# Ascend-Research/HeadPoseEstimation-WHENet

Hardware: NVIDIA H100
Metric: head-crops/sec @224x224 bf16 (higher is better)
Workload: dtype bf16

## Files before the change

### headposeestimation-whenet_b200/csrc/kernels_dwse.cuh

```cuda
#pragma once
#include <cuda.h>

#include "kernels_fused.cuh"

namespace whenet {
namespace fused {

struct alignas(64) DwSeParams {
    CUtensorMap tmE;
    CUtensorMap tmW;
    CUtensorMap tmX;
    CUtensorMap tmWx;
    const float* b_exp;
    const float* b_dw;
    int* tflag;
    void* out;
    float* partial;
    const float *w_se1t, *b_se1, *w_se2, *b_se2;
    float* gate;
    int Cse;
    float inv_hw;
    int se_tail;
    int scale_out;
    int C, pad;
    int n_chunks, chunks_per_cta;
    int N;
    int tiles_x, Ho_img;
};

template <int KS, int S, int HIN>
struct DwSeGeom {
    static constexpr int HO = (HIN + S - 1) / S;
    static constexpr int R = 7;
    static constexpr int SPR = HO / R;
    static constexpr int NSTRIPS = HO * SPR;
    static constexpr int PW = (HO - 1) * S + KS;
    static constexpr int NCOL = (R - 1) * S + KS;
};

template <int KS, int S, int HIN, int CC>
struct DwSeThreads { static constexpr int value = ((DwSeGeom<KS, S, HIN>::NSTRIPS * (CC / 4)) + 31) / 32 * 32; };

template <int KS, int S, int HIN, int CC>
constexpr size_t dwse_smem(int C, int Cse) {
    using G = DwSeGeom<KS, S, HIN>;
    return (size_t)2 * ((G::PW * G::PW * CC * 2 + 127) / 128 * 128)
           + (size_t)2 * ((CC * 4 + KS * KS * CC * 2 + 127) / 128 * 128)
           + (size_t)2 * G::NSTRIPS * CC * 4
           + (size_t)(C + Cse + 32) * 4 + 256;
}

template <typename T, int KS, int S, int HIN, int CC>
__device__ __forceinline__ void dw_strip(uint32_t erow, uint32_t cst, int cv, T* dst, int C, uint32_t red) {
    using G = DwSeGeom<KS, S, HIN>;
    constexpr int PITCH = CC * 2;
    const float4 bq = lds_f4(cst + (uint32_t)cv * 16);
    const uint32_t cst_h = cst + (uint32_t)(CC * 4 + cv * 8);
    __half2 hacc[G::R][2];
#pragma unroll
    for (int r = 0; r < G::R; ++r) { hacc[r][0] = __float2half2_rn(0.f); hacc[r][1] = __float2half2_rn(0.f); }
#pragma unroll
    for (int ky = 0; ky < KS; ++ky) {
        __half2 wr[KS][2];
#pragma unroll
        for (int kx = 0; kx < KS; ++kx) {
            uint32_t w0, w1;
            lds64(cst_h + (uint32_t)((ky * KS + kx) * CC) * 2, w0, w1);
            wr[kx][0] = *reinterpret_cast<__half2*>(&w0); wr[kx][1] = *reinterpret_cast<__half2*>(&w1);
        }
#pragma unroll
        for (int col = 0; col < G::NCOL; ++col) {
            uint32_t a, b;
            lds64(erow + (uint32_t)(col * PITCH), a, b);
            const __half2 x01 = *reinterpret_cast<__half2*>(&a), x23 = *reinterpret_cast<__half2*>(&b);
#pragma unroll
            for (int r = 0; r < G::R; ++r) {
                const int kx = col - r * S;
                if (kx >= 0 && kx < KS) {
                    hacc[r][0] = __hfma2(x01, wr[kx][0], hacc[r][0]);
                    hacc[r][1] = __hfma2(x23, wr[kx][1], hacc[r][1]);
                }
            }
        }
        erow += G::PW * PITCH;
    }
    const float2 sc = make_float2(kDwScale, kDwScale);
    float sum[4] = {0.f, 0.f, 0.f, 0.f};
#pragma unroll
    for (int r = 0; r < G::R; ++r) {
        float2 a0 = make_float2(bq.x, bq.y), a1 = make_float2(bq.z, bq.w);
        ffma2(a0, __half22float2(hacc[r][0]), sc);
        ffma2(a1, __half22float2(hacc[r][1]), sc);
        a0.x = swish_from_half(a0.x); a0.y = swish_from_half(a0.y);
        a1.x = swish_from_half(a1.x); a1.y = swish_from_half(a1.y);
        sum[0] += a0.x; sum[1] += a0.y; sum[2] += a1.x; sum[3] += a1.y;
        uint2 o;
        o.x = pack2<T>(a0.x, a0.y);
        o.y = pack2<T>(a1.x, a1.y);
        *reinterpret_cast<uint2*>(dst + (long long)r * C) = o;
    }
    asm volatile("st.shared.v4.f32 [%0], {%1,%2,%3,%4};" ::"r"(red), "f"(sum[0]), "f"(sum[1]), "f"(sum[2]), "f"(sum[3]) : "memory");
}

template <int NSTRIPS, int CC>
__device__ __forceinline__ void squeeze_sums(uint32_t red, float* dst, float* means, float inv_hw, int lane) {
    for (int cc = lane; cc < CC; cc += 32) {
        const uint32_t r0 = red + (uint32_t)(cc * 4);
        float s4[4] = {0.f, 0.f, 0.f, 0.f};
#pragma unroll
        for (int y = 0; y < NSTRIPS; ++y) {
            float t;
            asm volatile("ld.shared.f32 %0, [%1];" : "=f"(t) : "r"(r0 + (uint32_t)(y * CC * 4)));
            s4[y & 3] += t;
        }
        const float tot = (s4[0] + s4[1]) + (s4[2] + s4[3]);
        dst[cc] = tot;
        if (means) means[cc] = tot * inv_hw;
    }
}

template <typename T, int NT, int HO>
__device__ __forceinline__ void se_tail_gate(const DwSeParams& p, int n, T* out_n, float* sM) {
    const int C = p.C;
    se_gate_fc<NT>(sM, sM + C, p.w_se1t, p.b_se1, p.w_se2, p.b_se2, p.gate + (long long)n * C, C, p.Cse, sM);
    __syncthreads();
    if (p.scale_out) {
        const int cv8 = C >> 3, total = HO * HO * cv8;
        const float inv_cv8 = 1.0f / (float)cv8;
        for (int v = threadIdx.x; v < total; v += NT) {
            const int c8 = (v - div_small(v, inv_cv8) * cv8) * 8;
            uint4* ptr = reinterpret_cast<uint4*>(out_n) + v;
            *ptr = tc::scale8s<T>(__ldcg(ptr), tc::smem_u32(sM + c8));
        }
    }
}

template <typename T, int KS, int S, int HIN, int CC, bool SPATIAL = false>
__global__ void __launch_bounds__((DwSeThreads<KS, S, HIN, CC>::value)) dwse_kernel(const __grid_constant__ DwSeParams p) {
    using G = DwSeGeom<KS, S, HIN>;
    constexpr int NT = DwSeThreads<KS, S, HIN, CC>::value;
    constexpr int NW = NT / 32;
    constexpr int CV = CC / 4;
    constexpr int PITCH = CC * 2;
    constexpr int TILE_TX = G::PW * G::PW * PITCH;
    constexpr int TILE_BYTES = (TILE_TX + 127) / 128 * 128;
    constexpr int CST_TX = CC * 4 + KS * KS * CC * 2;
    constexpr int CST_BYTES = (CST_TX + 127) / 128 * 128;
    constexpr int RED_BYTES = G::NSTRIPS * CC * 4;
    extern __shared__ __align__(128) uint8_t smem_dw[];
    __shared__ __align__(8) uint64_t bars[4];
    __shared__ int s_abort_mem;
    volatile int* s_abort = &s_abort_mem;
    const uint32_t s0 = (tc::smem_u32(smem_dw) + 127u) & ~127u;
    const uint32_t sT = s0, sC = sT + 2 * TILE_BYTES, sR = sC + 2 * CST_BYTES;
    float* const sM = reinterpret_cast<float*>(smem_dw + (sR + 2 * RED_BYTES - tc::smem_u32(smem_dw)));
    const uint32_t b_full = tc::smem_u32(&bars[0]), b_empty = tc::smem_u32(&bars[2]);

    const int tid = threadIdx.x, warp = tid >> 5, lane = tid & 31;
    const int n = blockIdx.x;
    const int C = p.C;
    const int ch_begin = blockIdx.y * p.chunks_per_cta;
    const int ch_end = min(p.n_chunks, ch_begin + p.chunks_per_cta);
    const int Ho_img = SPATIAL ? p.Ho_img : G::HO;
    T* const out_n = reinterpret_cast<T*>(p.out) + (long long)n * Ho_img * Ho_img * C;

    if (tid == 0) {
        tc::mbar_init(&bars[0], 1); tc::mbar_init(&bars[1], 1);
        tc::mbar_init(&bars[2], NW); tc::mbar_init(&bars[3], NW);
        s_abort_mem = 0;
        asm volatile("fence.mbarrier_init.release.cluster;" ::: "memory");
        asm volatile("prefetch.tensormap [%0];" ::"l"(&p.tmE) : "memory");
        asm volatile("prefetch.tensormap [%0];" ::"l"(&p.tmW) : "memory");
    }
    __syncthreads();

    auto issue = [&](int ch, int buf) {
        const int cbase = SPATIAL ? 0 : ch * CC;
        const uint32_t bar = b_full + 8 * buf;
        tc::mbar::arrive_expect_tx(bar, (uint32_t)(TILE_TX + CST_TX));
        if (SPATIAL) {
            const int ty = ch / p.tiles_x, tx = ch - ty * p.tiles_x;
            tc::mbar::tma_4d(sT + buf * TILE_BYTES, &p.tmE, 0, tx * G::HO * S - p.pad, ty * G::HO * S - p.pad, n, bar);
        } else
            tc::mbar::tma_4d(sT + buf * TILE_BYTES, &p.tmE, cbase, -p.pad, -p.pad, n, bar);
        tc::mbar::tma_2d(sC + buf * CST_BYTES + CC * 4, &p.tmW, cbase, 0, bar);
        asm volatile("cp.async.bulk.shared::cluster.global.mbarrier::complete_tx::bytes [%0], [%1], %2, [%3];"
                     ::"r"(sC + buf * CST_BYTES), "l"(p.b_dw + cbase), "r"((uint32_t)(CC * 4)), "r"(bar) : "memory");
    };

    const int strip = tid / CV, cv = tid - strip * CV;
    const bool active = strip < G::NSTRIPS;
    const int oy = strip / G::SPR, ox0 = (strip - oy * G::SPR) * G::R;
    const uint32_t win = (uint32_t)(((oy * S) * G::PW + ox0 * S) * PITCH + cv * 8);

    if (tid == 0) {
        issue(ch_begin, 0);
        if (ch_begin + 1 < ch_end) issue(ch_begin + 1, 1);
    }

    for (int ch = ch_begin; ch < ch_end; ++ch) {
        const int it = ch - ch_begin, buf = it & 1;
        const uint32_t par = (uint32_t)(it >> 1) & 1u;
        tc::mbar::wait(b_full + 8 * buf, par, s_abort, p.tflag);
        if (active && !*s_abort) {
            T* dst;
            if (SPATIAL) {
                const int ty = ch / p.tiles_x, tx = ch - ty * p.tiles_x;
                dst = out_n + ((long long)(ty * G::HO + oy) * Ho_img + tx * G::HO + ox0) * C + cv * 4;
            } else
                dst = out_n + ((long long)oy * G::HO + ox0) * C + ch * CC + cv * 4;
            dw_strip<T, KS, S, HIN, CC>(sT + buf * TILE_BYTES + win, sC + buf * CST_BYTES, cv, dst, C,
                                        sR + (uint32_t)(buf * RED_BYTES + (strip * CC + cv * 4) * 4));
        }
        tc::mbar::arrive_warp(b_empty + 8 * buf);
        if (warp == 0) {
            tc::mbar::wait(b_empty + 8 * buf, par, s_abort, p.tflag);
            if (SPATIAL) squeeze_sums<G::NSTRIPS, CC>(sR + buf * RED_BYTES, p.partial + ((long long)n * p.n_chunks + ch) * C, nullptr, 0.f, lane);
            else squeeze_sums<G::NSTRIPS, CC>(sR + buf * RED_BYTES, p.partial + (long long)n * C + ch * CC, p.se_tail ? sM + ch * CC : nullptr, p.inv_hw, lane);
            __syncwarp();
            if (lane == 0 && ch + 2 < ch_end) issue(ch + 2, buf);
        }
    }
    __syncthreads();
    if (!SPATIAL && p.se_tail) se_tail_gate<T, NT, G::HO>(p, n, out_n, sM);
}

template <int KS, int S, int HIN, int CC, int CIN>
struct DwSeX {
    using G = DwSeGeom<KS, S, HIN>;
    static constexpr int NT = 256;
    static constexpr int NKB = (CIN + 63) / 64;
    static constexpr int KSTEPS = (CIN + 15) / 16;
    static constexpr int PIX = HIN * HIN;
    static constexpr int HALVES = (PIX + 63) / 64;
    static constexpr int XROWS = (PIX + 7) / 8 * 8;
    static_assert(HALVES == 4 || HALVES == 1, "14x14 or 7x7 maps");
    static constexpr int HPW = HALVES == 4 ? 2 : 1;
    static constexpr int NWG = HALVES == 4 ? CC : CC / 2;
    static_assert(NWG % 16 == 0 && NWG <= 128, "wgmma width");
    static_assert(G::NSTRIPS * (CC / 4) <= NT, "one depthwise strip per thread");
    static constexpr uint32_t X_KB = XROWS * 128, X_BYTES = NKB * X_KB;
    static constexpr uint32_t W_KB = CC * 128, W_BYTES = NKB * W_KB;
    static constexpr uint32_t TILE_BYTES = (G::PW * G::PW * CC * 2 + 127) / 128 * 128;
    static constexpr uint32_t CST_TX = CC * 4 + KS * KS * CC * 2;
    static constexpr uint32_t CST_BYTES = (CST_TX + 127) / 128 * 128;
    static constexpr uint32_t RED_BYTES = G::NSTRIPS * CC * 4;
    static constexpr uint32_t OFF_W = X_BYTES, OFF_T = OFF_W + 2 * W_BYTES, OFF_C = OFF_T + 2 * TILE_BYTES;
    static constexpr uint32_t OFF_R = OFF_C + 2 * CST_BYTES, OFF_M = OFF_R + 2 * RED_BYTES;
    static_assert((X_KB | W_KB | OFF_W | OFF_T) % 1024 == 0, "SWIZZLE_128B operands sit on 1024-byte boundaries");
    static constexpr size_t smem(int C, int Cse) { return (size_t)OFF_M + (size_t)(C + Cse + 32) * 4 + 1024; }
    static constexpr int CTAS_PER_SM = 2 * ((size_t)OFF_M + 4096 + 1024 + 1024) <= 228 * 1024 ? 2 : 1;
};

template <int KS, int S, int HIN, int CC, int CIN>
__global__ void __launch_bounds__(256, (DwSeX<KS, S, HIN, CC, CIN>::CTAS_PER_SM)) dwse_x_kernel(const __grid_constant__ DwSeParams p) {
    using X = DwSeX<KS, S, HIN, CC, CIN>;
    using G = typename X::G;
    using T = __nv_bfloat16;
    constexpr int NT = X::NT;
    constexpr int CV = CC / 4;
    extern __shared__ uint8_t smem_dwx[];
    __shared__ __align__(8) uint64_t bars[5];
    __shared__ int s_abort_mem;
    volatile int* s_abort = &s_abort_mem;
    const uint32_t s0 = (tc::smem_u32(smem_dwx) + 1023u) & ~1023u;
    const uint32_t sX = s0, sW = s0 + X::OFF_W, sT = s0 + X::OFF_T, sC = s0 + X::OFF_C, sR = s0 + X::OFF_R;
    float* const sM = reinterpret_cast<float*>(smem_dwx + (s0 + X::OFF_M - tc::smem_u32(smem_dwx)));
    const uint32_t b_x = tc::smem_u32(&bars[0]), b_w = b_x + 8, b_c = b_x + 24;

    const int tid = threadIdx.x, warp = tid >> 5, lane = tid & 31;
    const int wg = tid >> 7, wq = warp & 3;
    const int n = blockIdx.x;
    const int C = p.C, n_chunks = p.n_chunks;
    T* const out_n = reinterpret_cast<T*>(p.out) + (long long)n * G::HO * G::HO * C;

    if (tid == 0) {
        for (int i = 0; i < 5; ++i) tc::mbar_init(&bars[i], 1);
        s_abort_mem = 0;
        asm volatile("fence.mbarrier_init.release.cluster;" ::: "memory");
        asm volatile("prefetch.tensormap [%0];" ::"l"(&p.tmX) : "memory");
        asm volatile("prefetch.tensormap [%0];" ::"l"(&p.tmWx) : "memory");
        asm volatile("prefetch.tensormap [%0];" ::"l"(&p.tmW) : "memory");
    }
    for (uint32_t o = (uint32_t)tid * 16; o < 2 * X::TILE_BYTES; o += NT * 16) sts128(sT + o, make_uint4(0, 0, 0, 0));
    __syncthreads();

    auto issue_w = [&](int j) {
        const uint32_t bar = b_w + 8 * (j & 1);
        tc::mbar::arrive_expect_tx(bar, X::W_BYTES);
        for (int kb = 0; kb < X::NKB; ++kb) tc::mbar::tma_2d(sW + (j & 1) * X::W_BYTES + kb * X::W_KB, &p.tmWx, kb * 64, j * CC, bar);
    };
    auto issue_c = [&](int j) {
        const uint32_t bar = b_c + 8 * (j & 1), dst = sC + (j & 1) * X::CST_BYTES;
        tc::mbar::arrive_expect_tx(bar, X::CST_TX);
        tc::mbar::tma_2d(dst + CC * 4, &p.tmW, j * CC, 0, bar);
        asm volatile("cp.async.bulk.shared::cluster.global.mbarrier::complete_tx::bytes [%0], [%1], %2, [%3];"
                     ::"r"(dst), "l"(p.b_dw + j * CC), "r"((uint32_t)(CC * 4)), "r"(bar) : "memory");
    };
    if (tid == 0) {
        tc::mbar::arrive_expect_tx(b_x, X::X_BYTES);
        for (int kb = 0; kb < X::NKB; ++kb) tc::mbar::tma_2d(sX + kb * X::X_KB, &p.tmX, kb * 64, n * X::PIX, b_x);
        issue_w(0); issue_c(0);
        if (n_chunks > 1) { issue_w(1); issue_c(1); }
    }

    float acc[X::HPW][X::NWG / 2];
    auto mma = [&](int j) {
        tc::mbar::wait(b_x, 0, s_abort, p.tflag);
        tc::mbar::wait(b_w + 8 * (j & 1), (uint32_t)(j >> 1) & 1u, s_abort, p.tflag);
        const uint32_t wb = sW + (j & 1) * X::W_BYTES;
#pragma unroll
        for (int h = 0; h < X::HPW; ++h) {
            if constexpr (X::HALVES == 4) tc::wg_mma_m64<true, X::NWG>(acc[h], sX + (uint32_t)(wg * X::HPW + h) * 64 * 128, X::X_KB, wb, X::W_KB, X::KSTEPS);
            else tc::wg_mma_m64<true, X::NWG>(acc[h], sX, X::X_KB, wb + (uint32_t)wg * X::NWG * 128, X::W_KB, X::KSTEPS);
        }
    };
    auto epilogue = [&](int j) {
        const uint32_t tile = sT + (j & 1) * X::TILE_BYTES;
        const int c0 = X::HALVES == 4 ? 0 : wg * X::NWG;
        float2 bias[X::NWG / 8];
#pragma unroll
        for (int i = 0; i < X::NWG / 8; ++i) {
            const float* b = p.b_exp + j * CC + c0 + 8 * i + 2 * (lane & 3);
            bias[i] = make_float2(0.5f * __ldg(b), 0.5f * __ldg(b + 1));
        }
#pragma unroll
        for (int h = 0; h < X::HPW; ++h)
#pragma unroll
            for (int e = 0; e < 2; ++e) {
                const int pix = 64 * (X::HALVES == 4 ? wg * X::HPW + h : 0) + 16 * wq + (lane >> 2) + 8 * e;
                if (pix >= X::PIX) continue;
                const int y = pix / HIN, x = pix - y * HIN;
                const uint32_t prow = tile + (uint32_t)(((y + p.pad) * G::PW + x + p.pad) * CC + c0) * 2;
#pragma unroll
                for (int i = 0; i < X::NWG / 8; ++i) {
                    const int c = 8 * i + 2 * (lane & 3);
                    const float o0 = swish_from_half(fmaf(acc[h][4 * i + 2 * e], 0.5f, bias[i].x));
                    const float o1 = swish_from_half(fmaf(acc[h][4 * i + 2 * e + 1], 0.5f, bias[i].y));
                    asm volatile("st.shared.b32 [%0], %1;" ::"r"(prow + (uint32_t)c * 2), "r"(pack2<__half>(o0, o1)) : "memory");
                }
            }
    };

    const int strip = tid / CV, cv = tid - strip * CV;
    const bool active = strip < G::NSTRIPS;
    const int oy = strip / G::SPR, ox0 = (strip - oy * G::SPR) * G::R;
    const uint32_t win = (uint32_t)(((oy * S) * G::PW + ox0 * S) * CC * 2 + cv * 8);

    auto depthwise = [&](int j) {
        tc::mbar::wait(b_c + 8 * (j & 1), (uint32_t)(j >> 1) & 1u, s_abort, p.tflag);
        if (active && !*s_abort)
            dw_strip<T, KS, S, HIN, CC>(sT + (j & 1) * X::TILE_BYTES + win, sC + (j & 1) * X::CST_BYTES, cv,
                                        out_n + ((long long)oy * G::HO + ox0) * C + j * CC + cv * 4, C,
                                        sR + (uint32_t)((j & 1) * X::RED_BYTES + (strip * CC + cv * 4) * 4));
    };
    auto close = [&](int j) {
        if (warp == 0)
            squeeze_sums<G::NSTRIPS, CC>(sR + (j & 1) * X::RED_BYTES, p.partial + (long long)n * C + j * CC,
                                         p.se_tail ? sM + j * CC : nullptr, p.inv_hw, lane);
        if (tid == 0) {
            if (j + 3 < n_chunks) issue_w(j + 3);
            if (j + 2 < n_chunks) issue_c(j + 2);
        }
    };

    mma(0);
    tc::wg_wait<0>();
    epilogue(0);
    __syncthreads();
    if (tid == 0 && 2 < n_chunks) issue_w(2);
    for (int j = 0; j + 1 < n_chunks; ++j) {
        mma(j + 1);
        depthwise(j);
        tc::wg_wait<0>();
        epilogue(j + 1);
        __syncthreads();
        close(j);
    }
    depthwise(n_chunks - 1);
    __syncthreads();
    close(n_chunks - 1);
    __syncthreads();
    if (p.se_tail) se_tail_gate<T, NT, G::HO>(p, n, out_n, sM);
}

inline int dwse_chunk(int k, int s, int hin, int C) {
    if (hin == 14 && s == 1 && (k == 3 || k == 5) && C % 32 == 0) return 32;
    if (hin == 14 && s == 2 && k == 5 && C % 96 == 0) return 96;
    if (hin == 7 && s == 1 && (k == 3 || k == 5) && C % 128 == 0) return 128;
    return 0;
}

template <typename T>
int launch_dwse(cudaStream_t stream, DwSeParams p, int k, int s, int hin, int n_crops, int split) {
    const int CCr = dwse_chunk(k, s, hin, p.C);
    if (!CCr) return 1;
    p.N = n_crops;
    p.n_chunks = p.C / CCr;
    if (split < 1) split = 1;
    if (split > p.n_chunks) split = p.n_chunks;
    p.chunks_per_cta = (p.n_chunks + split - 1) / split;
    const int gy = (p.n_chunks + p.chunks_per_cta - 1) / p.chunks_per_cta;
    if (gy > 1) { p.se_tail = 0; p.scale_out = 0; }
#define DWSE(KS, S, HIN, CC)                                                                                              \
    do {                                                                                                                  \
        auto kfn = dwse_kernel<T, KS, S, HIN, CC>;                                                                        \
        const size_t smem = dwse_smem<KS, S, HIN, CC>(p.C, p.Cse);                                                        \
        if (cudaFuncSetAttribute(kfn, cudaFuncAttributeMaxDynamicSharedMemorySize, (int)smem) != cudaSuccess) return -1;  \
        kfn<<<dim3(n_crops, gy), DwSeThreads<KS, S, HIN, CC>::value, smem, stream>>>(p);                                    \
        return 0;                                                                                                         \
    } while (0)
    if (hin == 14 && s == 1 && k == 3) DWSE(3, 1, 14, 32);
    if (hin == 14 && s == 1 && k == 5) DWSE(5, 1, 14, 32);
    if (hin == 14 && s == 2 && k == 5) DWSE(5, 2, 14, 96);
    if (hin == 7 && s == 1 && k == 5) DWSE(5, 1, 7, 128);
    if (hin == 7 && s == 1 && k == 3) DWSE(3, 1, 7, 128);
#undef DWSE
    return 1;
}


template <typename T>
int launch_dwse_x(cudaStream_t stream, DwSeParams p, int k, int s, int hin, int cin, int n_crops) {
    static_assert(std::is_same<T, __nv_bfloat16>::value, "the on-chip expand runs the bf16 wgmma");
    const int CCr = dwse_chunk(k, s, hin, p.C);
    if (!CCr) return 1;
    p.N = n_crops;
    p.n_chunks = p.C / CCr;
    p.chunks_per_cta = p.n_chunks;
#define DWSEX(KS, S, HIN, CC, CIN)                                                                                        \
    do {                                                                                                                  \
        auto kfn = dwse_x_kernel<KS, S, HIN, CC, CIN>;                                                                    \
        const size_t smem = DwSeX<KS, S, HIN, CC, CIN>::smem(p.C, p.Cse);                                                 \
        if (cudaFuncSetAttribute(kfn, cudaFuncAttributeMaxDynamicSharedMemorySize, (int)smem) != cudaSuccess) return -1;  \
        kfn<<<n_crops, DwSeX<KS, S, HIN, CC, CIN>::NT, smem, stream>>>(p);                                                \
        return 0;                                                                                                         \
    } while (0)
    if (CCr == 32 && hin == 14 && s == 1 && k == 3 && cin == 80) DWSEX(3, 1, 14, 32, 80);
    if (CCr == 32 && hin == 14 && s == 1 && k == 5 && cin == 80) DWSEX(5, 1, 14, 32, 80);
    if (CCr == 32 && hin == 14 && s == 1 && k == 5 && cin == 112) DWSEX(5, 1, 14, 32, 112);
    if (CCr == 96 && hin == 14 && s == 2 && k == 5 && cin == 112) DWSEX(5, 2, 14, 96, 112);
    if (CCr == 128 && hin == 7 && s == 1 && k == 5 && cin == 192) DWSEX(5, 1, 7, 128, 192);
    if (CCr == 128 && hin == 7 && s == 1 && k == 3 && cin == 192) DWSEX(3, 1, 7, 128, 192);
#undef DWSEX
    return 1;
}

template <typename T>
int launch_dwse_spatial(cudaStream_t stream, DwSeParams p, int H, int n_crops, int split) {
    if (p.C != 32 || H % 14) return 1;
    p.N = n_crops;
    p.tiles_x = H / 14; p.Ho_img = H;
    p.n_chunks = p.tiles_x * p.tiles_x;
    if (split < 1) split = 1;
    if (split > p.n_chunks) split = p.n_chunks;
    p.chunks_per_cta = (p.n_chunks + split - 1) / split;
    const int gy = (p.n_chunks + p.chunks_per_cta - 1) / p.chunks_per_cta;
    p.se_tail = 0; p.scale_out = 0;
    auto kfn = dwse_kernel<T, 3, 1, 14, 32, true>;
    const size_t smem = dwse_smem<3, 1, 14, 32>(0, 0);
    if (cudaFuncSetAttribute(kfn, cudaFuncAttributeMaxDynamicSharedMemorySize, (int)smem) != cudaSuccess) return -1;
    kfn<<<dim3(n_crops, gy), DwSeThreads<3, 1, 14, 32>::value, smem, stream>>>(p);
    return 0;
}

}
}
```

Before: 87540.

## Make fused expand-depthwise-SE kernel persistent with cross-crop prefetch and chunk rotation

Turns the fused expand+depthwise+SE kernel into a persistent kernel. The grid is sized to occupancy times SM count, and each CTA loops over crops, prefetching the next crop's input tile and the next weight chunks while the current crop is still finishing. Each CTA also starts at a chunk offset based on blockIdx so concurrent CTAs read different weight chunks. This aims to hide per-CTA launch and prologue latency and smooth weight traffic, at the cost of more complex barrier phase tracking and an added host-side occupancy query on every launch.

```diff
diff --git a/headposeestimation-whenet_b200/csrc/kernels_dwse.cuh b/headposeestimation-whenet_b200/csrc/kernels_dwse.cuh
--- a/headposeestimation-whenet_b200/csrc/kernels_dwse.cuh
+++ b/headposeestimation-whenet_b200/csrc/kernels_dwse.cuh
@@ -270,9 +270,9 @@
 
     const int tid = threadIdx.x, warp = tid >> 5, lane = tid & 31;
     const int wg = tid >> 7, wq = warp & 3;
-    const int n = blockIdx.x;
     const int C = p.C, n_chunks = p.n_chunks;
-    T* const out_n = reinterpret_cast<T*>(p.out) + (long long)n * G::HO * G::HO * C;
+    const int rot = blockIdx.x % n_chunks;
+    auto chunk = [&](int k) { return k + rot < n_chunks ? k + rot : k + rot - n_chunks; };
 
     if (tid == 0) {
         for (int i = 0; i < 5; ++i) tc::mbar_init(&bars[i], 1);
@@ -285,38 +285,40 @@
     for (uint32_t o = (uint32_t)tid * 16; o < 2 * X::TILE_BYTES; o += NT * 16) sts128(sT + o, make_uint4(0, 0, 0, 0));
     __syncthreads();
 
-    auto issue_w = [&](int j) {
-        const uint32_t bar = b_w + 8 * (j & 1);
+    auto issue_x = [&](int n) {
+        tc::mbar::arrive_expect_tx(b_x, X::X_BYTES);
+        for (int kb = 0; kb < X::NKB; ++kb) tc::mbar::tma_2d(sX + kb * X::X_KB, &p.tmX, kb * 64, n * X::PIX, b_x);
+    };
+    auto issue_w = [&](int g, int j) {
+        const uint32_t bar = b_w + 8 * (g & 1);
         tc::mbar::arrive_expect_tx(bar, X::W_BYTES);
-        for (int kb = 0; kb < X::NKB; ++kb) tc::mbar::tma_2d(sW + (j & 1) * X::W_BYTES + kb * X::W_KB, &p.tmWx, kb * 64, j * CC, bar);
-    };
-    auto issue_c = [&](int j) {
-        const uint32_t bar = b_c + 8 * (j & 1), dst = sC + (j & 1) * X::CST_BYTES;
+        for (int kb = 0; kb < X::NKB; ++kb) tc::mbar::tma_2d(sW + (g & 1) * X::W_BYTES + kb * X::W_KB, &p.tmWx, kb * 64, j * CC, bar);
+    };
+    auto issue_c = [&](int g, int j) {
+        const uint32_t bar = b_c + 8 * (g & 1), dst = sC + (g & 1) * X::CST_BYTES;
         tc::mbar::arrive_expect_tx(bar, X::CST_TX);
         tc::mbar::tma_2d(dst + CC * 4, &p.tmW, j * CC, 0, bar);
         asm volatile("cp.async.bulk.shared::cluster.global.mbarrier::complete_tx::bytes [%0], [%1], %2, [%3];"
                      ::"r"(dst), "l"(p.b_dw + j * CC), "r"((uint32_t)(CC * 4)), "r"(bar) : "memory");
     };
     if (tid == 0) {
-        tc::mbar::arrive_expect_tx(b_x, X::X_BYTES);
-        for (int kb = 0; kb < X::NKB; ++kb) tc::mbar::tma_2d(sX + kb * X::X_KB, &p.tmX, kb * 64, n * X::PIX, b_x);
-        issue_w(0); issue_c(0);
-        if (n_chunks > 1) { issue_w(1); issue_c(1); }
+        issue_x(blockIdx.x);
+        issue_w(0, chunk(0)); issue_c(0, chunk(0));
+        issue_w(1, chunk(1)); issue_c(1, chunk(1));
     }
 
     float acc[X::HPW][X::NWG / 2];
-    auto mma = [&](int j) {
-        tc::mbar::wait(b_x, 0, s_abort, p.tflag);
-        tc::mbar::wait(b_w + 8 * (j & 1), (uint32_t)(j >> 1) & 1u, s_abort, p.tflag);
-        const uint32_t wb = sW + (j & 1) * X::W_BYTES;
+    auto mma = [&](int g) {
+        tc::mbar::wait(b_w + 8 * (g & 1), (uint32_t)(g >> 1) & 1u, s_abort, p.tflag);
+        const uint32_t wb = sW + (g & 1) * X::W_BYTES;
 #pragma unroll
         for (int h = 0; h < X::HPW; ++h) {
             if constexpr (X::HALVES == 4) tc::wg_mma_m64<true, X::NWG>(acc[h], sX + (uint32_t)(wg * X::HPW + h) * 64 * 128, X::X_KB, wb, X::W_KB, X::KSTEPS);
             else tc::wg_mma_m64<true, X::NWG>(acc[h], sX, X::X_KB, wb + (uint32_t)wg * X::NWG * 128, X::W_KB, X::KSTEPS);
         }
     };
-    auto epilogue = [&](int j) {
-        const uint32_t tile = sT + (j & 1) * X::TILE_BYTES;
+    auto epilogue = [&](int g, int j) {
+        const uint32_t tile = sT + (g & 1) * X::TILE_BYTES;
         const int c0 = X::HALVES == 4 ? 0 : wg * X::NWG;
         float2 bias[X::NWG / 8];
 #pragma unroll
@@ -346,42 +348,51 @@
     const bool active = strip < G::NSTRIPS;
     const int oy = strip / G::SPR, ox0 = (strip - oy * G::SPR) * G::R;
     const uint32_t win = (uint32_t)(((oy * S) * G::PW + ox0 * S) * CC * 2 + cv * 8);
-
-    auto depthwise = [&](int j) {
-        tc::mbar::wait(b_c + 8 * (j & 1), (uint32_t)(j >> 1) & 1u, s_abort, p.tflag);
+    const int dst0 = (oy * G::HO + ox0) * C + cv * 4;
+
+    auto depthwise = [&](int g, int j, int n) {
+        tc::mbar::wait(b_c + 8 * (g & 1), (uint32_t)(g >> 1) & 1u, s_abort, p.tflag);
         if (active && !*s_abort)
-            dw_strip<T, KS, S, HIN, CC>(sT + (j & 1) * X::TILE_BYTES + win, sC + (j & 1) * X::CST_BYTES, cv,
-                                        out_n + ((long long)oy * G::HO + ox0) * C + j * CC + cv * 4, C,
-                                        sR + (uint32_t)((j & 1) * X::RED_BYTES + (strip * CC + cv * 4) * 4));
-    };
-    auto close = [&](int j) {
+            dw_strip<T, KS, S, HIN, CC>(sT + (g & 1) * X::TILE_BYTES + win, sC + (g & 1) * X::CST_BYTES, cv,
+                                        reinterpret_cast<T*>(p.out) + (long long)n * G::HO * G::HO * C + (dst0 + j * CC), C,
+                                        sR + (uint32_t)((g & 1) * X::RED_BYTES + (strip * CC + cv * 4) * 4));
+    };
+    auto close = [&](int g, int k, int n, bool more) {
+        const int j = chunk(k);
         if (warp == 0)
-            squeeze_sums<G::NSTRIPS, CC>(sR + (j & 1) * X::RED_BYTES, p.partial + (long long)n * C + j * CC,
+            squeeze_sums<G::NSTRIPS, CC>(sR + (g & 1) * X::RED_BYTES, p.partial + (long long)n * C + j * CC,
                                          p.se_tail ? sM + j * CC : nullptr, p.inv_hw, lane);
-        if (tid == 0) {
-            if (j + 3 < n_chunks) issue_w(j + 3);
-            if (j + 2 < n_chunks) issue_c(j + 2);
-        }
-    };
-
-    mma(0);
-    tc::wg_wait<0>();
-    epilogue(0);
-    __syncthreads();
-    if (tid == 0 && 2 < n_chunks) issue_w(2);
-    for (int j = 0; j + 1 < n_chunks; ++j) {
-        mma(j + 1);
-        depthwise(j);
+        if (tid == 0 && (more || k + 2 < n_chunks)) issue_c(g + 2, chunk((k + 2) % n_chunks));
+    };
+
+    for (int n = blockIdx.x, g0 = 0;; n += gridDim.x, g0 += n_chunks) {
+        const bool more = n + (int)gridDim.x < p.N;
+        tc::mbar::wait(b_x, (uint32_t)(g0 / n_chunks) & 1u, s_abort, p.tflag);
+        mma(g0);
         tc::wg_wait<0>();
-        epilogue(j + 1);
+        epilogue(g0, chunk(0));
         __syncthreads();
-        close(j);
-    }
-    depthwise(n_chunks - 1);
-    __syncthreads();
-    close(n_chunks - 1);
-    __syncthreads();
-    if (p.se_tail) se_tail_gate<T, NT, G::HO>(p, n, out_n, sM);
+        if (tid == 0 && (more || 2 < n_chunks)) issue_w(g0 + 2, chunk(2 % n_chunks));
+        for (int k = 0; k + 1 < n_chunks; ++k) {
+            const int g = g0 + k;
+            mma(g + 1);
+            depthwise(g, chunk(k), n);
+            tc::wg_wait<0>();
+            epilogue(g + 1, chunk(k + 1));
+            __syncthreads();
+            if (tid == 0) {
+                if (more && k + 2 == n_chunks) issue_x(n + gridDim.x);
+                if (more || k + 3 < n_chunks) issue_w(g + 3, chunk((k + 3) % n_chunks));
+            }
+            close(g, k, n, more);
+        }
+        depthwise(g0 + n_chunks - 1, chunk(n_chunks - 1), n);
+        __syncthreads();
+        close(g0 + n_chunks - 1, n_chunks - 1, n, more);
+        if (__syncthreads_or(*s_abort)) return;
+        if (p.se_tail) se_tail_gate<T, NT, G::HO>(p, n, reinterpret_cast<T*>(p.out) + (long long)n * G::HO * G::HO * C, sM);
+        if (!more) return;
+    }
 }
 
 inline int dwse_chunk(int k, int s, int hin, int C) {
@@ -424,16 +435,21 @@
 int launch_dwse_x(cudaStream_t stream, DwSeParams p, int k, int s, int hin, int cin, int n_crops) {
     static_assert(std::is_same<T, __nv_bfloat16>::value, "the on-chip expand runs the bf16 wgmma");
     const int CCr = dwse_chunk(k, s, hin, p.C);
-    if (!CCr) return 1;
+    if (!CCr || p.C / CCr < 2) return 1;
     p.N = n_crops;
     p.n_chunks = p.C / CCr;
     p.chunks_per_cta = p.n_chunks;
 #define DWSEX(KS, S, HIN, CC, CIN)                                                                                        \
     do {                                                                                                                  \
         auto kfn = dwse_x_kernel<KS, S, HIN, CC, CIN>;                                                                    \
+        constexpr int NT = DwSeX<KS, S, HIN, CC, CIN>::NT;                                                                \
         const size_t smem = DwSeX<KS, S, HIN, CC, CIN>::smem(p.C, p.Cse);                                                 \
         if (cudaFuncSetAttribute(kfn, cudaFuncAttributeMaxDynamicSharedMemorySize, (int)smem) != cudaSuccess) return -1;  \
-        kfn<<<n_crops, DwSeX<KS, S, HIN, CC, CIN>::NT, smem, stream>>>(p);                                                \
+        int dev = 0, sms = 0, per_sm = 0;                                                                                 \
+        if (cudaGetDevice(&dev) != cudaSuccess || cudaDeviceGetAttribute(&sms, cudaDevAttrMultiProcessorCount, dev) != cudaSuccess || \
+            cudaOccupancyMaxActiveBlocksPerMultiprocessor(&per_sm, kfn, NT, smem) != cudaSuccess || per_sm < 1)            \
+            return -1;                                                                                                    \
+        kfn<<<std::min(n_crops, per_sm * sms), NT, smem, stream>>>(p);                                                    \
         return 0;                                                                                                         \
     } while (0)
     if (CCr == 32 && hin == 14 && s == 1 && k == 3 && cin == 80) DWSEX(3, 1, 14, 32, 80);
```

Result: no change. 87710, median of 6 (+0.2%).
